# jolibrain/joliGEN

Hardware: AMD Instinct MI355X
Metric: train images/sec at 256x256 (DDPM UNet step) (higher is better)
Workload: dtype bf16; 1 GPU; palette_model DDPM, efficient UNet unet_mha ngf64 mults[1,2,4,8] res_blocks[2,2,2,2] mid-attn 16x32, 256x256, batch 32/GPU, inpainting synthetic masks, AdamW+EMA, iter_size 1 (example_ddpm_noglasses2glasses.json + SURVEY Appendix C overrides); global_batch=32, per_gpu_batch=32, image_size=256, efficient=True, parallelism=dp1, n_ranks_seen=1

## Files before the change

### joligen_amd/csrc/conv1x1.hip

```cpp
#include <stdlib.h>

#include "conv_params.h"

namespace {

__device__ __forceinline__ float act_rt(float u, int act) {
  return act == JG_ACT_SILU ? silu_f(u) : act == JG_ACT_RELU ? fmaxf(u, 0.f) : act == JG_ACT_LRELU ? (u > 0.f ? u : 0.2f * u) : u;
}

template <typename T, int PAIRS, int KS, bool APPLY = false, bool GNB = false>
__global__ __launch_bounds__(256, 2) void conv1x1_stream_kernel(ConvP p, int ntiles) {
  __shared__ __attribute__((aligned(16))) float s_ab[APPLY ? 4 * 2 * KS * 32 : (GNB ? 4 * 5 * PAIRS * 32 : 4)];
  const int lane = threadIdx.x & 63;
  const int a = lane & 15, g = lane >> 4;
  const int n0 = blockIdx.y * (PAIRS * 32);
  const T* __restrict__ x = (const T*)p.x;
  const T* __restrict__ w = (const T*)p.w;
  const T* __restrict__ res = (const T*)p.res;
  T* __restrict__ y = (T*)p.y;

  uint4 wf[PAIRS][2][KS];
#pragma unroll
  for (int pr = 0; pr < PAIRS; ++pr)
#pragma unroll
    for (int hf = 0; hf < 2; ++hf) {
      const int n = n0 + pr * 32 + (a >> 2) * 8 + hf * 4 + (a & 3);
#pragma unroll
      for (int ks = 0; ks < KS; ++ks) wf[pr][hf][ks] = *reinterpret_cast<const uint4*>(w + (long)n * p.ldw + ks * 32 + g * 8);
    }
  float bs[PAIRS][8];
#pragma unroll
  for (int pr = 0; pr < PAIRS; ++pr)
#pragma unroll
    for (int j = 0; j < 8; ++j) bs[pr][j] = (!GNB && p.bias) ? p.bias[n0 + pr * 32 + g * 8 + j] : 0.f;

  const int wave = blockIdx.x * 4 + (threadIdx.x >> 6), nwaves = gridDim.x * 4;
  auto load_tile = [&](int t, uint4* xf) {
    const T* px = x + ((long)t * 16 + a) * p.ldx + g * 8;
#pragma unroll
    for (int ks = 0; ks < KS; ++ks) xf[ks] = *reinterpret_cast<const uint4*>(px + ks * 32);
  };
  const bool do_apply = APPLY && blockIdx.y == 0;
  float* wab = s_ab + (threadIdx.x >> 6) * (APPLY ? 2 * KS * 32 : (GNB ? 5 * PAIRS * 32 : 1));
  const int tiles_per_img = (p.Ho * p.Wo) >> 4;
  int cur_b = -1;
  constexpr int PF = KS <= 2 ? 4 : (KS <= 4 ? 2 : 1);
  uint4 ring[PF][KS];
#pragma unroll
  for (int s = 0; s < PF; ++s)
    if (wave + s * nwaves < ntiles) load_tile(wave + s * nwaves, ring[s]);
  for (int base = wave; base < ntiles; base += PF * nwaves) {
#pragma unroll
    for (int s = 0; s < PF; ++s) {
      const int t = base + s * nwaves;
      if (t >= ntiles) break;
      const long prow = ((long)t * 16 + a);
      if (GNB) {
        const int b = t / tiles_per_img;
        if (b != cur_b) {
          cur_b = b;
          constexpr int NC = PAIRS * 32;
          for (int c = lane; c < NC; c += 64) {
            const long row = (long)b * p.N + n0 + c;
            wab[c] = p.bab[row * 2];
            wab[NC + c] = p.bab[row * 2 + 1];
            wab[2 * NC + c] = p.bpqr[row * 3];
            wab[3 * NC + c] = p.bpqr[row * 3 + 1];
            wab[4 * NC + c] = p.bpqr[row * 3 + 2];
          }
        }
      }
      uint4 rf[PAIRS];
      if (res) {
#pragma unroll
        for (int pr = 0; pr < PAIRS; ++pr) rf[pr] = *reinterpret_cast<const uint4*>(res + prow * p.ldres + n0 + pr * 32 + g * 8);
      }
      f32x4 acc[PAIRS][2];
#pragma unroll
      for (int pr = 0; pr < PAIRS; ++pr) {
        acc[pr][0] = acc[pr][1] = (f32x4){0.f, 0.f, 0.f, 0.f};
#pragma unroll
        for (int ks = 0; ks < KS; ++ks) {
          acc[pr][0] = Mfma<T>::run(wf[pr][0][ks], ring[s][ks], acc[pr][0]);
          acc[pr][1] = Mfma<T>::run(wf[pr][1][ks], ring[s][ks], acc[pr][1]);
        }
      }
      if (do_apply) {
        const int b = t / tiles_per_img;
        if (b != cur_b) {
          cur_b = b;
          const float* src = p.aab + (long)b * (2 * KS * 32);
          for (int i = lane; i < 2 * KS * 32 / 4; i += 64) reinterpret_cast<float4*>(wab)[i] = reinterpret_cast<const float4*>(src)[i];
        }
        T* ay = (T*)p.ay + prow * p.lday + g * 8;
#pragma unroll
        for (int ks = 0; ks < KS; ++ks) {
          float f[8];
          unpack8<T>(ring[s][ks], f);
          const float4* c4 = reinterpret_cast<const float4*>(wab + (ks * 32 + g * 8) * 2);
#pragma unroll
          for (int k4 = 0; k4 < 4; ++k4) {
            const float4 c = c4[k4];
            const float u0 = c.x * f[2 * k4] + c.y, u1 = c.z * f[2 * k4 + 1] + c.w;
            f[2 * k4] = p.aact == JG_ACT_SILU ? silu_f(u0) : act_rt(u0, p.aact);
            f[2 * k4 + 1] = p.aact == JG_ACT_SILU ? silu_f(u1) : act_rt(u1, p.aact);
          }
          *reinterpret_cast<uint4*>(ay + ks * 32) = pack8<T>(f);
        }
      }
      const int tn = t + PF * nwaves;
      if (tn < ntiles) load_tile(tn, ring[s]);
#pragma unroll
      for (int pr = 0; pr < PAIRS; ++pr) {
        float o[8] = {acc[pr][0][0], acc[pr][0][1], acc[pr][0][2], acc[pr][0][3], acc[pr][1][0], acc[pr][1][1], acc[pr][1][2], acc[pr][1][3]};
        float r8[8];
        if (res) unpack8<T>(rf[pr], r8);
#pragma unroll
        for (int j = 0; j < 8; ++j) o[j] = GNB ? p.alpha * o[j] : p.alpha * o[j] + bs[pr][j] + (res ? p.res_scale * r8[j] : 0.f);
        if (GNB) {
          constexpr int NC = PAIRS * 32;
          const int cl = pr * 32 + g * 8, cg = n0 + cl;
          float fx[8], fd[8], ca[8], cb[8], cP[8], cQ[8], cR[8];
          unpack8<T>(*reinterpret_cast<const uint4*>((const T*)p.bgx + prow * p.bldgx + cg), fx);
          unpack8<T>(*reinterpret_cast<const uint4*>((const T*)p.bgdy + prow * p.bldgdy + cg), fd);
#pragma unroll
          for (int h = 0; h < 2; ++h) {
            *reinterpret_cast<float4*>(ca + 4 * h) = *reinterpret_cast<const float4*>(wab + cl + 4 * h);
            *reinterpret_cast<float4*>(cb + 4 * h) = *reinterpret_cast<const float4*>(wab + NC + cl + 4 * h);
            *reinterpret_cast<float4*>(cP + 4 * h) = *reinterpret_cast<const float4*>(wab + 2 * NC + cl + 4 * h);
            *reinterpret_cast<float4*>(cQ + 4 * h) = *reinterpret_cast<const float4*>(wab + 3 * NC + cl + 4 * h);
            *reinterpret_cast<float4*>(cR + 4 * h) = *reinterpret_cast<const float4*>(wab + 4 * NC + cl + 4 * h);
          }
#pragma unroll
          for (int j = 0; j < 8; ++j) {
            float du = fd[j];
            if (p.bact != JG_ACT_NONE) du *= act_grad_rt(ca[j] * fx[j] + cb[j], p.bact);
            o[j] += du * cP[j] + fx[j] * cQ[j] + cR[j];
          }
          if (p.badd1) {
            float fa[8];
            unpack8<T>(*reinterpret_cast<const uint4*>((const T*)p.badd1 + prow * p.bldadd1 + cg), fa);
#pragma unroll
            for (int j = 0; j < 8; ++j) o[j] += p.bsc1 * fa[j];
          }
          if (p.badd2) {
            float fa[8];
            unpack8<T>(*reinterpret_cast<const uint4*>((const T*)p.badd2 + prow * p.bldadd2 + cg), fa);
#pragma unroll
            for (int j = 0; j < 8; ++j) o[j] += p.bsc2 * fa[j];
          }
        }
        *reinterpret_cast<uint4*>(y + prow * p.ldy + n0 + pr * 32 + g * 8) = pack8<T>(o);
        if (GNB) __builtin_amdgcn_sched_barrier(0);
      }
    }
  }
}

template <typename T, int PAIRS>
__global__ __launch_bounds__(256, 2) void conv3x3_c8_stream_kernel(ConvP p, int ntiles) {
  constexpr int KS = 3;
  const int lane = threadIdx.x & 63;
  const int a = lane & 15, g = lane >> 4;
  const int n0 = blockIdx.y * (PAIRS * 32);
  const T* __restrict__ x = (const T*)p.x;
  const T* __restrict__ w = (const T*)p.w;
  const T* __restrict__ res = (const T*)p.res;
  T* __restrict__ y = (T*)p.y;
  const uint4 zero4 = make_uint4(0u, 0u, 0u, 0u);
  uint4 wf[PAIRS][2][KS];
#pragma unroll
  for (int pr = 0; pr < PAIRS; ++pr)
#pragma unroll
    for (int hf = 0; hf < 2; ++hf) {
      const int n = n0 + pr * 32 + (a >> 2) * 8 + hf * 4 + (a & 3);
#pragma unroll
      for (int ks = 0; ks < KS; ++ks) {
        const int tap = ks * 4 + g;
        wf[pr][hf][ks] = tap < 9 ? *reinterpret_cast<const uint4*>(w + (long)n * p.ldw + tap * 8) : zero4;
      }
    }
  float bs[PAIRS][8];
#pragma unroll
  for (int pr = 0; pr < PAIRS; ++pr)
#pragma unroll
    for (int j = 0; j < 8; ++j) bs[pr][j] = p.bias ? p.bias[n0 + pr * 32 + g * 8 + j] : 0.f;
  const int wave = blockIdx.x * 4 + (threadIdx.x >> 6), nwaves = gridDim.x * 4;
  auto load_tile = [&](int t, uint4* xf) {
    const long pix = (long)t * 16 + a;
    const int px = pix % p.W, py = (pix / p.W) % p.H;
#pragma unroll
    for (int ks = 0; ks < KS; ++ks) {
      const int tap = ks * 4 + g;
      const int dy = tap / 3 - 1, dx = tap % 3 - 1;
      const bool ok = tap < 9 && (unsigned)(py + dy) < (unsigned)p.H && (unsigned)(px + dx) < (unsigned)p.W;
      xf[ks] = ok ? *reinterpret_cast<const uint4*>(x + (pix + (long)dy * p.W + dx) * 8) : zero4;
    }
  };
  const int per = (ntiles + nwaves - 1) / nwaves;
  const int t0 = wave * per, t1 = min(ntiles, t0 + per);
  const int tiles_per_img = (p.H * p.W) >> 4;
  float s1[PAIRS][8], s2[PAIRS][8];
#pragma unroll
  for (int pr = 0; pr < PAIRS; ++pr)
#pragma unroll
    for (int j = 0; j < 8; ++j) s1[pr][j] = s2[pr][j] = 0.f;
  int cur_b = t0 < t1 ? t0 / tiles_per_img : 0;
  auto flush = [&](int b) {
    float* base = p.stats + ((long)(b * p.nslots + wave % p.nslots) * p.ldstats) * 2;
#pragma unroll
    for (int pr = 0; pr < PAIRS; ++pr)
#pragma unroll
      for (int j = 0; j < 8; ++j) {
        float u = s1[pr][j], v = s2[pr][j];
#pragma unroll
        for (int o = 1; o < 16; o <<= 1) {
          u += __shfl_xor(u, o);
          v += __shfl_xor(v, o);
        }
        if (a == 0) {
          atomicAdd(base + (n0 + pr * 32 + g * 8 + j) * 2, u);
          atomicAdd(base + (n0 + pr * 32 + g * 8 + j) * 2 + 1, v);
        }
        s1[pr][j] = s2[pr][j] = 0.f;
      }
  };
  constexpr int PF = 2;
  uint4 ring[PF][KS];
#pragma unroll
  for (int s = 0; s < PF; ++s)
    if (t0 + s < t1) load_tile(t0 + s, ring[s]);
  for (int base = t0; base < t1; base += PF) {
#pragma unroll
    for (int s = 0; s < PF; ++s) {
      const int t = base + s;
      if (t < t1) {
        const long prow = ((long)t * 16 + a);
        if (p.stats) {
          const int b = t / tiles_per_img;
          if (b != cur_b) {
            flush(cur_b);
            cur_b = b;
          }
        }
        f32x4 acc[PAIRS][2];
#pragma unroll
        for (int pr = 0; pr < PAIRS; ++pr) {
          acc[pr][0] = acc[pr][1] = (f32x4){0.f, 0.f, 0.f, 0.f};
#pragma unroll
          for (int ks = 0; ks < KS; ++ks) {
            acc[pr][0] = Mfma<T>::run(wf[pr][0][ks], ring[s][ks], acc[pr][0]);
            acc[pr][1] = Mfma<T>::run(wf[pr][1][ks], ring[s][ks], acc[pr][1]);
          }
        }
        if (t + PF < t1) load_tile(t + PF, ring[s]);
#pragma unroll
        for (int pr = 0; pr < PAIRS; ++pr) {
          float o[8] = {acc[pr][0][0], acc[pr][0][1], acc[pr][0][2], acc[pr][0][3], acc[pr][1][0], acc[pr][1][1], acc[pr][1][2], acc[pr][1][3]};
          float r8[8];
          if (res) unpack8<T>(*reinterpret_cast<const uint4*>(res + prow * p.ldres + n0 + pr * 32 + g * 8), r8);
#pragma unroll
          for (int j = 0; j < 8; ++j) {
            o[j] = p.alpha * o[j] + bs[pr][j] + (res ? p.res_scale * r8[j] : 0.f);
            s1[pr][j] += o[j];
            s2[pr][j] += o[j] * o[j];
          }
          *reinterpret_cast<uint4*>(y + prow * p.ldy + n0 + pr * 32 + g * 8) = pack8<T>(o);
        }
      }
    }
  }
  if (p.stats && t0 < t1) flush(cur_b);
}

template <typename T>
void launch_c8(const ConvP& p, hipStream_t st) {
  const int ntiles = p.M / 16;
  const int ngroups = p.N / 64;
  int bx = (ntiles + 3) / 4;
  const int cap = 256 * 8 / ngroups > 64 ? 256 * 8 / ngroups : 64;
  if (bx > cap) bx = cap;
  jg_note_kernel("conv3x3_c8_stream_kernel");
  hipLaunchKernelGGL((conv3x3_c8_stream_kernel<T, 2>), dim3(bx, ngroups), dim3(256), 0, st, p, ntiles);
}


template <typename T, int PAIRS, int KS>
void launch_1x1(const ConvP& p, hipStream_t st) {
  const int ntiles = p.M / 16;
  const int ngroups = p.N / (PAIRS * 32);
  int bx = (ntiles + 3) / 4;
  const int cap = 256 * 8 / ngroups > 64 ? 256 * 8 / ngroups : 64;
  if (bx > cap) bx = cap;
  if (p.aab) {
    jg_note_kernel("conv1x1_stream_kernel+gn_apply");
    hipLaunchKernelGGL((conv1x1_stream_kernel<T, PAIRS, KS, true>), dim3(bx, ngroups), dim3(256), 0, st, p, ntiles);
  } else if (p.bgx) {
    jg_note_kernel("conv1x1_stream_kernel+gn_bwd_apply");
    hipLaunchKernelGGL((conv1x1_stream_kernel<T, PAIRS, KS, false, true>), dim3(bx, ngroups), dim3(256), 0, st, p, ntiles);
  } else {
    jg_note_kernel("conv1x1_stream_kernel");
    hipLaunchKernelGGL((conv1x1_stream_kernel<T, PAIRS, KS>), dim3(bx, ngroups), dim3(256), 0, st, p, ntiles);
  }
}

template <typename T, int PAIRS, int KS>
void launch_1x1_plain(const ConvP& p, hipStream_t st) {
  const int ntiles = p.M / 16;
  const int ngroups = p.N / (PAIRS * 32);
  int bx = (ntiles + 3) / 4;
  const int cap = 256 * 8 / ngroups > 64 ? 256 * 8 / ngroups : 64;
  if (bx > cap) bx = cap;
  jg_note_kernel("conv1x1_stream_kernel");
  hipLaunchKernelGGL((conv1x1_stream_kernel<T, PAIRS, KS>), dim3(bx, ngroups), dim3(256), 0, st, p, ntiles);
}

template <typename T>
bool dispatch_1x1(const ConvP& p, hipStream_t st) {
  const int ks = p.Cin / 32;
  const bool wide = p.N % 128 == 0;
  if (!p.aab && !p.bgx) {
    if (ks == 1) {
      if (wide) launch_1x1_plain<T, 4, 1>(p, st);
      else if (p.N % 64 == 0) launch_1x1_plain<T, 2, 1>(p, st);
      else launch_1x1_plain<T, 1, 1>(p, st);
      return true;
    }
    if (p.N % 64) {
      switch (ks) {
        case 2: launch_1x1_plain<T, 1, 2>(p, st); return true;
        case 4: launch_1x1_plain<T, 1, 4>(p, st); return true;
        case 8: launch_1x1_plain<T, 1, 8>(p, st); return true;
        default: return false;
      }
    }
  } else if (ks == 1 || p.N % 64) {
    return false;
  }
  switch (ks) {
    case 2: wide ? launch_1x1<T, 4, 2>(p, st) : launch_1x1<T, 2, 2>(p, st); return true;
    case 4: launch_1x1<T, 2, 4>(p, st); return true;
    case 6: launch_1x1<T, 2, 6>(p, st); return true;
    case 8: launch_1x1<T, 2, 8>(p, st); return true;
    default: return false;
  }
}

}

bool jg_conv1x1_try(int dtype, const ConvP& p, int nbatch, hipStream_t st) {
  if (p.res_up || p.x_up || p.y_pool) return false;
  const bool off = jg_tune(JG_TUNE_CONV1X1) == 0;
  if (off && !p.aab && !p.bgx) return false;
  if (!p.aab && !p.bgx && nbatch == 1 && p.nh == 1 && p.R == 3 && p.S == 3 && p.pad == 1 && p.stride == 1 && !p.out_f32 && !(p.stats && p.stats_mode) && !p.reflect &&
      p.Cin == 8 && ((p.H * p.W) & 15) == 0 &&
      p.ldx == 8 && p.ldw == 72 && p.N % 64 == 0 && !(p.M & 15) && p.H == p.Ho && p.W == p.Wo && p.ldy % 8 == 0 && (!p.res || p.ldres % 8 == 0) &&
      (long)p.M >= 65536) {
    if (dtype == JG_F16) launch_c8<f16_t>(p, st);
    else if (dtype == JG_BF16) launch_c8<bf16_t>(p, st);
    else return false;
    return true;
  }
  if (nbatch != 1 || p.nh != 1 || p.R != 1 || p.S != 1 || p.pad != 0 || p.stride != 1 || p.out_f32 || p.stats || p.reflect) return false;
  if (p.Cin % 32 || p.Cin > 256 || p.N % 32 || (p.M & 15)) return false;
  if (p.ldx % 8 || p.ldy % 8 || p.ldw % 8 || (p.res && p.ldres % 8)) return false;
  if ((long)p.M < 65536) return false;
  if (!p.aab && !p.bgx && p.Cin >= 256 && p.N >= 256 && jg_tune(JG_TUNE_CONV1X1) < 2) return false;
  if (dtype == JG_F16) return dispatch_1x1<f16_t>(p, st);
  if (dtype == JG_BF16) return dispatch_1x1<bf16_t>(p, st);
  return false;
}
```

Measured before the change: 673.8 images/sec.

## Split fused GN 1x1 conv into contiguous-run kernel with prefetched coefficients

Adds a separate conv1x1 kernel for the GroupNorm-apply and GN-backward fused paths. Each wave now processes a contiguous run of tiles instead of a grid stride, so per-image coefficients change rarely and the next image's set is loaded ahead in registers. Epilogue operands are loaded before the MFMAs and held in place with scheduling barriers, activations are specialised at compile time, large weight fragment sets are staged in LDS, and KS=4 wide backward uses PAIRS=4. The cost is more code and register or LDS pressure, and contiguous runs may change load balance and memory access patterns.

```diff
diff --git a/joligen_amd/csrc/conv1x1.hip b/joligen_amd/csrc/conv1x1.hip
--- a/joligen_amd/csrc/conv1x1.hip
+++ b/joligen_amd/csrc/conv1x1.hip
@@ -8,9 +8,8 @@
   return act == JG_ACT_SILU ? silu_f(u) : act == JG_ACT_RELU ? fmaxf(u, 0.f) : act == JG_ACT_LRELU ? (u > 0.f ? u : 0.2f * u) : u;
 }
 
-template <typename T, int PAIRS, int KS, bool APPLY = false, bool GNB = false>
+template <typename T, int PAIRS, int KS>
 __global__ __launch_bounds__(256, 2) void conv1x1_stream_kernel(ConvP p, int ntiles) {
-  __shared__ __attribute__((aligned(16))) float s_ab[APPLY ? 4 * 2 * KS * 32 : (GNB ? 4 * 5 * PAIRS * 32 : 4)];
   const int lane = threadIdx.x & 63;
   const int a = lane & 15, g = lane >> 4;
   const int n0 = blockIdx.y * (PAIRS * 32);
@@ -32,7 +31,7 @@
 #pragma unroll
   for (int pr = 0; pr < PAIRS; ++pr)
 #pragma unroll
-    for (int j = 0; j < 8; ++j) bs[pr][j] = (!GNB && p.bias) ? p.bias[n0 + pr * 32 + g * 8 + j] : 0.f;
+    for (int j = 0; j < 8; ++j) bs[pr][j] = p.bias ? p.bias[n0 + pr * 32 + g * 8 + j] : 0.f;
 
   const int wave = blockIdx.x * 4 + (threadIdx.x >> 6), nwaves = gridDim.x * 4;
   auto load_tile = [&](int t, uint4* xf) {
@@ -40,10 +39,6 @@
 #pragma unroll
     for (int ks = 0; ks < KS; ++ks) xf[ks] = *reinterpret_cast<const uint4*>(px + ks * 32);
   };
-  const bool do_apply = APPLY && blockIdx.y == 0;
-  float* wab = s_ab + (threadIdx.x >> 6) * (APPLY ? 2 * KS * 32 : (GNB ? 5 * PAIRS * 32 : 1));
-  const int tiles_per_img = (p.Ho * p.Wo) >> 4;
-  int cur_b = -1;
   constexpr int PF = KS <= 2 ? 4 : (KS <= 4 ? 2 : 1);
   uint4 ring[PF][KS];
 #pragma unroll
@@ -55,21 +50,6 @@
       const int t = base + s * nwaves;
       if (t >= ntiles) break;
       const long prow = ((long)t * 16 + a);
-      if (GNB) {
-        const int b = t / tiles_per_img;
-        if (b != cur_b) {
-          cur_b = b;
-          constexpr int NC = PAIRS * 32;
-          for (int c = lane; c < NC; c += 64) {
-            const long row = (long)b * p.N + n0 + c;
-            wab[c] = p.bab[row * 2];
-            wab[NC + c] = p.bab[row * 2 + 1];
-            wab[2 * NC + c] = p.bpqr[row * 3];
-            wab[3 * NC + c] = p.bpqr[row * 3 + 1];
-            wab[4 * NC + c] = p.bpqr[row * 3 + 2];
-          }
-        }
-      }
       uint4 rf[PAIRS];
       if (res) {
 #pragma unroll
@@ -85,13 +65,152 @@
           acc[pr][1] = Mfma<T>::run(wf[pr][1][ks], ring[s][ks], acc[pr][1]);
         }
       }
+      const int tn = t + PF * nwaves;
+      if (tn < ntiles) load_tile(tn, ring[s]);
+#pragma unroll
+      for (int pr = 0; pr < PAIRS; ++pr) {
+        float o[8] = {acc[pr][0][0], acc[pr][0][1], acc[pr][0][2], acc[pr][0][3], acc[pr][1][0], acc[pr][1][1], acc[pr][1][2], acc[pr][1][3]};
+        float r8[8];
+        if (res) unpack8<T>(rf[pr], r8);
+#pragma unroll
+        for (int j = 0; j < 8; ++j) o[j] = p.alpha * o[j] + bs[pr][j] + (res ? p.res_scale * r8[j] : 0.f);
+        *reinterpret_cast<uint4*>(y + prow * p.ldy + n0 + pr * 32 + g * 8) = pack8<T>(o);
+      }
+    }
+  }
+}
+
+constexpr int ACT_RT = -1;
+
+template <typename T, int PAIRS, int KS, bool GNB, int ACT>
+__global__ __launch_bounds__(256, 2) void conv1x1_stream_runs_kernel(ConvP p, int ntiles) {
+  constexpr bool WLDS = KS >= 6 || (GNB && PAIRS == 4);
+  constexpr int NC = PAIRS * 32, NCOEF = GNB ? 5 * NC : 2 * KS * 32, NFRAG = PAIRS * 2 * KS;
+  __shared__ __attribute__((aligned(16))) float s_ab[4 * NCOEF];
+  __shared__ uint4 s_w[WLDS ? NFRAG * 64 : 1];
+  const int lane = threadIdx.x & 63, wv = __builtin_amdgcn_readfirstlane(threadIdx.x >> 6);
+  const int a = lane & 15, g = lane >> 4;
+  const int n0 = blockIdx.y * NC;
+  const T* __restrict__ x = (const T*)p.x;
+  const T* __restrict__ w = (const T*)p.w;
+  const T* __restrict__ res = (const T*)p.res;
+  T* __restrict__ y = (T*)p.y;
+
+  auto load_wfrag = [&](int pr, int hf, int ks) {
+    const int n = n0 + pr * 32 + (a >> 2) * 8 + hf * 4 + (a & 3);
+    return *reinterpret_cast<const uint4*>(w + (long)n * p.ldw + ks * 32 + g * 8);
+  };
+  uint4 wf[WLDS ? 1 : NFRAG];
+  if constexpr (WLDS) {
+    for (int f = wv; f < NFRAG; f += 4) s_w[f * 64 + lane] = load_wfrag(f / (2 * KS), (f / KS) & 1, f % KS);
+    __syncthreads();
+  } else {
+#pragma unroll
+    for (int f = 0; f < NFRAG; ++f) wf[f] = load_wfrag(f / (2 * KS), (f / KS) & 1, f % KS);
+  }
+  float bs[PAIRS][8];
+#pragma unroll
+  for (int pr = 0; pr < PAIRS; ++pr)
+#pragma unroll
+    for (int j = 0; j < 8; ++j) bs[pr][j] = (!GNB && p.bias) ? p.bias[n0 + pr * 32 + g * 8 + j] : 0.f;
+
+  const int wave = blockIdx.x * 4 + wv, nwaves = gridDim.x * 4;
+  const int t0 = (int)((long)wave * ntiles / nwaves), t1 = (int)((long)(wave + 1) * ntiles / nwaves);
+  if (t0 >= t1) return;
+  auto load_tile = [&](int t, uint4* xf) {
+    const T* px = x + ((long)t * 16 + a) * p.ldx + g * 8;
+#pragma unroll
+    for (int ks = 0; ks < KS; ++ks) xf[ks] = *reinterpret_cast<const uint4*>(px + ks * 32);
+  };
+  const bool do_apply = !GNB && blockIdx.y == 0;
+  const bool coefs = GNB || do_apply;
+  const bool has1 = GNB && p.badd1, has2 = GNB && p.badd2;
+  float* wab = s_ab + wv * NCOEF;
+
+  constexpr int NQ = 2 * KS * 32 / 4;
+  struct Coef { float a, b, P, Q, R; } k0, k1;
+  float4 q0, q1;
+  auto coef_load = [&](int b) {
+    if constexpr (GNB) {
+      const float* ab = p.bab + ((long)b * p.N + n0 + lane) * 2;
+      const float* pqr = p.bpqr + ((long)b * p.N + n0 + lane) * 3;
+      k0 = Coef{ab[0], ab[1], pqr[0], pqr[1], pqr[2]};
+      if (NC > 64) k1 = Coef{ab[128], ab[129], pqr[192], pqr[193], pqr[194]};
+    } else {
+      const float4* src = reinterpret_cast<const float4*>(p.aab + (long)b * (2 * KS * 32));
+      if (lane < NQ) q0 = src[lane];
+      if (64 + lane < NQ) q1 = src[64 + lane];
+    }
+  };
+  auto coef_store = [&]() {
+    if constexpr (GNB) {
+      float* d = wab + lane;
+      d[0] = k0.a, d[NC] = k0.b, d[2 * NC] = k0.P, d[3 * NC] = k0.Q, d[4 * NC] = k0.R;
+      if (NC > 64) d[64] = k1.a, d[NC + 64] = k1.b, d[2 * NC + 64] = k1.P, d[3 * NC + 64] = k1.Q, d[4 * NC + 64] = k1.R;
+    } else {
+      if (lane < NQ) reinterpret_cast<float4*>(wab)[lane] = q0;
+      if (64 + lane < NQ) reinterpret_cast<float4*>(wab)[64 + lane] = q1;
+    }
+  };
+
+  const int tiles_per_img = (p.Ho * p.Wo) >> 4;
+  int img = t0 / tiles_per_img;
+  int tb = (img + 1) * tiles_per_img;
+  if (coefs) coef_load(img);
+  constexpr int PF = KS <= 2 ? 4 : (KS <= 4 ? 2 : 1);
+  uint4 ring[PF][KS];
+#pragma unroll
+  for (int s = 0; s < PF; ++s)
+    if (t0 + s < t1) load_tile(t0 + s, ring[s]);
+  if (coefs) {
+    coef_store();
+    if (tb < t1) coef_load(img + 1);
+  }
+  for (int base = t0; base < t1; base += PF) {
+#pragma unroll
+    for (int s = 0; s < PF; ++s) {
+      const int t = base + s;
+      if (t >= t1) break;
+      const long prow = ((long)t * 16 + a);
+      if (coefs && t == tb) {
+        coef_store();
+        ++img;
+        tb += tiles_per_img;
+        if (tb < t1) coef_load(img + 1);
+      }
+      uint4 rf[PAIRS], egx[PAIRS], egd[PAIRS], ea1[PAIRS], ea2[PAIRS];
+      const int cg = n0 + g * 8;
+      if constexpr (GNB) {
+#pragma unroll
+        for (int pr = 0; pr < PAIRS; ++pr) {
+          egx[pr] = *reinterpret_cast<const uint4*>((const T*)p.bgx + prow * p.bldgx + cg + pr * 32);
+          egd[pr] = *reinterpret_cast<const uint4*>((const T*)p.bgdy + prow * p.bldgdy + cg + pr * 32);
+        }
+        if (has1) {
+#pragma unroll
+          for (int pr = 0; pr < PAIRS; ++pr) ea1[pr] = *reinterpret_cast<const uint4*>((const T*)p.badd1 + prow * p.bldadd1 + cg + pr * 32);
+        }
+        if (has2) {
+#pragma unroll
+          for (int pr = 0; pr < PAIRS; ++pr) ea2[pr] = *reinterpret_cast<const uint4*>((const T*)p.badd2 + prow * p.bldadd2 + cg + pr * 32);
+        }
+      } else if (res) {
+#pragma unroll
+        for (int pr = 0; pr < PAIRS; ++pr) rf[pr] = *reinterpret_cast<const uint4*>(res + prow * p.ldres + cg + pr * 32);
+      }
+      __builtin_amdgcn_sched_barrier(0);
+      f32x4 acc[PAIRS][2];
+#pragma unroll
+      for (int pr = 0; pr < PAIRS; ++pr) {
+        acc[pr][0] = acc[pr][1] = (f32x4){0.f, 0.f, 0.f, 0.f};
+#pragma unroll
+        for (int ks = 0; ks < KS; ++ks) {
+          const int f0 = (pr * 2) * KS + ks, f1 = (pr * 2 + 1) * KS + ks;
+          acc[pr][0] = Mfma<T>::run(WLDS ? s_w[f0 * 64 + lane] : wf[WLDS ? 0 : f0], ring[s][ks], acc[pr][0]);
+          acc[pr][1] = Mfma<T>::run(WLDS ? s_w[f1 * 64 + lane] : wf[WLDS ? 0 : f1], ring[s][ks], acc[pr][1]);
+        }
+      }
       if (do_apply) {
-        const int b = t / tiles_per_img;
-        if (b != cur_b) {
-          cur_b = b;
-          const float* src = p.aab + (long)b * (2 * KS * 32);
-          for (int i = lane; i < 2 * KS * 32 / 4; i += 64) reinterpret_cast<float4*>(wab)[i] = reinterpret_cast<const float4*>(src)[i];
-        }
         T* ay = (T*)p.ay + prow * p.lday + g * 8;
 #pragma unroll
         for (int ks = 0; ks < KS; ++ks) {
@@ -102,27 +221,41 @@
           for (int k4 = 0; k4 < 4; ++k4) {
             const float4 c = c4[k4];
             const float u0 = c.x * f[2 * k4] + c.y, u1 = c.z * f[2 * k4 + 1] + c.w;
-            f[2 * k4] = p.aact == JG_ACT_SILU ? silu_f(u0) : act_rt(u0, p.aact);
-            f[2 * k4 + 1] = p.aact == JG_ACT_SILU ? silu_f(u1) : act_rt(u1, p.aact);
+            f[2 * k4] = ACT == ACT_RT ? act_rt(u0, p.aact) : act_f<ACT>(u0);
+            f[2 * k4 + 1] = ACT == ACT_RT ? act_rt(u1, p.aact) : act_f<ACT>(u1);
           }
           *reinterpret_cast<uint4*>(ay + ks * 32) = pack8<T>(f);
         }
       }
-      const int tn = t + PF * nwaves;
-      if (tn < ntiles) load_tile(tn, ring[s]);
+      if (GNB) load_tile(t + PF < t1 ? t + PF : t, ring[s]);
+      else if (t + PF < t1) load_tile(t + PF, ring[s]);
+      __builtin_amdgcn_sched_barrier(0);
+      if constexpr (GNB) {
+#pragma unroll
+        for (int pr = 0; pr < PAIRS; ++pr) {
+          asm volatile("" : "+v"(egx[pr].x), "+v"(egx[pr].y), "+v"(egx[pr].z), "+v"(egx[pr].w));
+          asm volatile("" : "+v"(egd[pr].x), "+v"(egd[pr].y), "+v"(egd[pr].z), "+v"(egd[pr].w));
+        }
+        if (has1) {
+#pragma unroll
+          for (int pr = 0; pr < PAIRS; ++pr) asm volatile("" : "+v"(ea1[pr].x), "+v"(ea1[pr].y), "+v"(ea1[pr].z), "+v"(ea1[pr].w));
+        }
+        if (has2) {
+#pragma unroll
+          for (int pr = 0; pr < PAIRS; ++pr) asm volatile("" : "+v"(ea2[pr].x), "+v"(ea2[pr].y), "+v"(ea2[pr].z), "+v"(ea2[pr].w));
+        }
+      } else if (res) {
+#pragma unroll
+        for (int pr = 0; pr < PAIRS; ++pr) asm volatile("" : "+v"(rf[pr].x), "+v"(rf[pr].y), "+v"(rf[pr].z), "+v"(rf[pr].w));
+      }
 #pragma unroll
       for (int pr = 0; pr < PAIRS; ++pr) {
         float o[8] = {acc[pr][0][0], acc[pr][0][1], acc[pr][0][2], acc[pr][0][3], acc[pr][1][0], acc[pr][1][1], acc[pr][1][2], acc[pr][1][3]};
-        float r8[8];
-        if (res) unpack8<T>(rf[pr], r8);
-#pragma unroll
-        for (int j = 0; j < 8; ++j) o[j] = GNB ? p.alpha * o[j] : p.alpha * o[j] + bs[pr][j] + (res ? p.res_scale * r8[j] : 0.f);
-        if (GNB) {
-          constexpr int NC = PAIRS * 32;
-          const int cl = pr * 32 + g * 8, cg = n0 + cl;
+        if constexpr (GNB) {
+          const int cl = pr * 32 + g * 8;
           float fx[8], fd[8], ca[8], cb[8], cP[8], cQ[8], cR[8];
-          unpack8<T>(*reinterpret_cast<const uint4*>((const T*)p.bgx + prow * p.bldgx + cg), fx);
-          unpack8<T>(*reinterpret_cast<const uint4*>((const T*)p.bgdy + prow * p.bldgdy + cg), fd);
+          unpack8<T>(egx[pr], fx);
+          unpack8<T>(egd[pr], fd);
 #pragma unroll
           for (int h = 0; h < 2; ++h) {
             *reinterpret_cast<float4*>(ca + 4 * h) = *reinterpret_cast<const float4*>(wab + cl + 4 * h);
@@ -133,24 +266,34 @@
           }
 #pragma unroll
           for (int j = 0; j < 8; ++j) {
+            o[j] = p.alpha * o[j];
             float du = fd[j];
-            if (p.bact != JG_ACT_NONE) du *= act_grad_rt(ca[j] * fx[j] + cb[j], p.bact);
+            if (ACT == ACT_RT) {
+              if (p.bact != JG_ACT_NONE) du *= act_grad_rt(ca[j] * fx[j] + cb[j], p.bact);
+            } else if (ACT != JG_ACT_NONE) {
+              du *= act_grad_f<ACT>(ca[j] * fx[j] + cb[j]);
+            }
             o[j] += du * cP[j] + fx[j] * cQ[j] + cR[j];
           }
-          if (p.badd1) {
+          if (has1) {
             float fa[8];
-            unpack8<T>(*reinterpret_cast<const uint4*>((const T*)p.badd1 + prow * p.bldadd1 + cg), fa);
+            unpack8<T>(ea1[pr], fa);
 #pragma unroll
             for (int j = 0; j < 8; ++j) o[j] += p.bsc1 * fa[j];
           }
-          if (p.badd2) {
+          if (has2) {
             float fa[8];
-            unpack8<T>(*reinterpret_cast<const uint4*>((const T*)p.badd2 + prow * p.bldadd2 + cg), fa);
+            unpack8<T>(ea2[pr], fa);
 #pragma unroll
             for (int j = 0; j < 8; ++j) o[j] += p.bsc2 * fa[j];
           }
-        }
-        *reinterpret_cast<uint4*>(y + prow * p.ldy + n0 + pr * 32 + g * 8) = pack8<T>(o);
+        } else {
+          float r8[8];
+          if (res) unpack8<T>(rf[pr], r8);
+#pragma unroll
+          for (int j = 0; j < 8; ++j) o[j] = p.alpha * o[j] + bs[pr][j] + (res ? p.res_scale * r8[j] : 0.f);
+        }
+        *reinterpret_cast<uint4*>(y + prow * p.ldy + cg + pr * 32) = pack8<T>(o);
         if (GNB) __builtin_amdgcn_sched_barrier(0);
       }
     }
@@ -285,34 +428,36 @@
 }
 
 
-template <typename T, int PAIRS, int KS>
-void launch_1x1(const ConvP& p, hipStream_t st) {
-  const int ntiles = p.M / 16;
-  const int ngroups = p.N / (PAIRS * 32);
+inline dim3 grid_1x1(int ntiles, int ngroups) {
   int bx = (ntiles + 3) / 4;
   const int cap = 256 * 8 / ngroups > 64 ? 256 * 8 / ngroups : 64;
   if (bx > cap) bx = cap;
-  if (p.aab) {
-    jg_note_kernel("conv1x1_stream_kernel+gn_apply");
-    hipLaunchKernelGGL((conv1x1_stream_kernel<T, PAIRS, KS, true>), dim3(bx, ngroups), dim3(256), 0, st, p, ntiles);
-  } else if (p.bgx) {
-    jg_note_kernel("conv1x1_stream_kernel+gn_bwd_apply");
-    hipLaunchKernelGGL((conv1x1_stream_kernel<T, PAIRS, KS, false, true>), dim3(bx, ngroups), dim3(256), 0, st, p, ntiles);
-  } else {
-    jg_note_kernel("conv1x1_stream_kernel");
-    hipLaunchKernelGGL((conv1x1_stream_kernel<T, PAIRS, KS>), dim3(bx, ngroups), dim3(256), 0, st, p, ntiles);
-  }
+  return dim3(bx, ngroups);
 }
 
 template <typename T, int PAIRS, int KS>
 void launch_1x1_plain(const ConvP& p, hipStream_t st) {
   const int ntiles = p.M / 16;
-  const int ngroups = p.N / (PAIRS * 32);
-  int bx = (ntiles + 3) / 4;
-  const int cap = 256 * 8 / ngroups > 64 ? 256 * 8 / ngroups : 64;
-  if (bx > cap) bx = cap;
   jg_note_kernel("conv1x1_stream_kernel");
-  hipLaunchKernelGGL((conv1x1_stream_kernel<T, PAIRS, KS>), dim3(bx, ngroups), dim3(256), 0, st, p, ntiles);
+  hipLaunchKernelGGL((conv1x1_stream_kernel<T, PAIRS, KS>), grid_1x1(ntiles, p.N / (PAIRS * 32)), dim3(256), 0, st, p, ntiles);
+}
+
+template <typename T, int PAIRS, int KS, bool GNB>
+void launch_1x1_runs(const ConvP& p, hipStream_t st) {
+  const int ntiles = p.M / 16;
+  const dim3 grid = grid_1x1(ntiles, p.N / (PAIRS * 32));
+  const int act = GNB ? p.bact : p.aact;
+  jg_note_kernel(GNB ? "conv1x1_stream_kernel+gn_bwd_apply" : "conv1x1_stream_kernel+gn_apply");
+  if (act == JG_ACT_SILU) hipLaunchKernelGGL((conv1x1_stream_runs_kernel<T, PAIRS, KS, GNB, JG_ACT_SILU>), grid, dim3(256), 0, st, p, ntiles);
+  else if (act == JG_ACT_NONE) hipLaunchKernelGGL((conv1x1_stream_runs_kernel<T, PAIRS, KS, GNB, JG_ACT_NONE>), grid, dim3(256), 0, st, p, ntiles);
+  else hipLaunchKernelGGL((conv1x1_stream_runs_kernel<T, PAIRS, KS, GNB, ACT_RT>), grid, dim3(256), 0, st, p, ntiles);
+}
+
+template <typename T, int PAIRS, int KS>
+void launch_1x1(const ConvP& p, hipStream_t st) {
+  if (p.aab) launch_1x1_runs<T, PAIRS, KS, false>(p, st);
+  else if (p.bgx) launch_1x1_runs<T, PAIRS, KS, true>(p, st);
+  else launch_1x1_plain<T, PAIRS, KS>(p, st);
 }
 
 template <typename T>
@@ -339,7 +484,10 @@
   }
   switch (ks) {
     case 2: wide ? launch_1x1<T, 4, 2>(p, st) : launch_1x1<T, 2, 2>(p, st); return true;
-    case 4: launch_1x1<T, 2, 4>(p, st); return true;
+    case 4:
+      if (wide && p.bgx) launch_1x1_runs<T, 4, 4, true>(p, st);
+      else launch_1x1<T, 2, 4>(p, st);
+      return true;
     case 6: launch_1x1<T, 2, 6>(p, st); return true;
     case 8: launch_1x1<T, 2, 8>(p, st); return true;
     default: return false;
```

After: 685.3 images/sec, median of 6. +1.7%, better.
